# Perception4D/LidarSlam

Hardware: AMD Instinct MI355X
Metric: LiDAR frames/sec (AddFrame end-to-end), VLS-128 scan (higher is better)
Workload: dtype f32+f64; 1 GPU; VLS-128 synthetic spinning scan, street canyon, 5 m/s, EgoMotion=MOTION_EXTRAPOLATION_AND_REGISTRATION, Undistortion=REFINED, library defaults; points_per_frame=255802, sequences=1, parallelism=1 sequence per GPU x 1, frames_resident_in_hbm=False

## Files before the change

include/lidarslam_amd.h:

```cpp
#ifndef LIDARSLAM_AMD_H
#define LIDARSLAM_AMD_H

#include <stddef.h>
#include <stdint.h>

#ifdef __cplusplus
extern "C" {
#endif

#define LSA_OK 0
#define LSA_E_NO_DEVICE (-1)
#define LSA_E_HIP (-2)
#define LSA_E_ARG (-3)
#define LSA_E_STATE (-4)
#define LSA_E_CAPACITY (-5)

#define LSA_EDGE 0
#define LSA_PLANE 1
#define LSA_BLOB 2

typedef struct lsa_point_t
{
  float x, y, z, w;
  double time;
// ... 118 lines not shown
int lsa_stage_target_ahead(lsa_ctx* ctx, int slot, int type, int m);
int lsa_drop_target_ahead(lsa_ctx* ctx, int slot, int type);
int lsa_staged_targets_adopted(const lsa_ctx* ctx);
int lsa_set_target_from_set(lsa_ctx* ctx, int slot, int type, int set);
int lsa_prepare_previous_targets(lsa_ctx* ctx, unsigned type_mask);
int lsa_prepared_targets_adopted(const lsa_ctx* ctx);
int lsa_target_size(const lsa_ctx* ctx, int slot, int type);
int lsa_download_target(lsa_ctx* ctx, int slot, int type, lsa_point_t* out, int capacity);
int lsa_set_target_cell_size(lsa_ctx* ctx, int slot, int type, float cell);
int lsa_set_knn_lanes(lsa_ctx* ctx, int type, int lanes);
int lsa_set_knn_rounds(lsa_ctx* ctx, int type, int rounds);

long long lsa_match_serial(const lsa_ctx* ctx, int type);
int lsa_match_histogram(lsa_ctx* ctx, int type, long long serial, int histogram[LSA_MATCH_NSTATUS]);
int lsa_match_types_undistorted(lsa_ctx* ctx, int slot, unsigned type_mask, const lsa_match_params_t* p, const double pose[16], int* histograms,
                                const double H0[16], const double H1[16], double t0, double t1);
int lsa_set_fused_match(lsa_ctx* ctx, int on);
int lsa_match_slow_queries(lsa_ctx* ctx);
int lsa_match_route_stats(lsa_ctx* ctx, int type, int out[8]);
int lsa_match_trace(lsa_ctx* ctx, unsigned long long* out, int blocks);
int lsa_match_exhaustive_queries(lsa_ctx* ctx);

int lsa_set_keypoints(lsa_ctx* ctx, int set, int type, const lsa_point_t* pts, int k);

int lsa_match(lsa_ctx* ctx, int slot, int type, int query_set, const lsa_match_params_t* params, const double pose[16],
              int histogram[LSA_MATCH_NSTATUS]);

int lsa_match_types(lsa_ctx* ctx, int slot, unsigned type_mask, int query_set, const lsa_match_params_t* params, const double pose[16],
                    int* histograms);

int lsa_overlap(lsa_ctx* ctx, unsigned type_mask, int interpolate, const double H0[16], const double H1[16], double t0, double t1, float sampling_ratio,
                const double leaf_size[3], float* overlap);

int lsa_download_match(lsa_ctx* ctx, int type, uint8_t* status, double* weights, double* records, int capacity);
int lsa_upload_match(lsa_ctx* ctx, int type, const uint8_t* status, const double* records, int n, double saturation);
#define LSA_KNN_MAX 16
int lsa_download_knn(lsa_ctx* ctx, int type, int* idx, float* d2, int* cnt, int capacity);

int lsa_accumulate(lsa_ctx* ctx, unsigned type_mask, const double w[6], int want_jacobian, double* cost, double g[6],
                   double H[36], int* n_valid);
int lsa_mailbox_active(const lsa_ctx* ctx);

int lsa_solve(lsa_ctx* ctx, unsigned type_mask, const double prior[16], int lm_max_iter, int two_d_mode, double optimized[16],
              int summary[4], double costs[2]);
typedef struct lsa_solve_result
{
  double pose[6];
  double initial_cost, final_cost;
  double cost, g[6], H[36];
  int num_successful_steps;
  int num_unsuccessful_steps;
  int num_iterations;
  int num_evaluations;
  int num_matches;
  int skipped;
  int termination;
  const char* message;
} lsa_solve_result_t;
int lsa_solve_device(lsa_ctx* ctx, unsigned type_mask, const double prior[6], int two_d_mode, int lm_max_iter, int min_matches,
                     lsa_solve_result_t* out);
int lsa_solve_device_begin(lsa_ctx* ctx, unsigned type_mask, const double prior[6], int two_d_mode, int lm_max_iter, int min_matches);
int lsa_solve_device_end(lsa_ctx* ctx, lsa_solve_result_t* out);
int lsa_solve_device_drop(lsa_ctx* ctx);

int lsa_icp_cancel(lsa_ctx* ctx, int ticket);
int lsa_icp_abandon(lsa_ctx* ctx);
int lsa_match_types_linked(lsa_ctx* ctx, int slot, unsigned type_mask, int query_set, const lsa_match_params_t* p, int undistort);
typedef struct lsa_icp_link
{
  int refine_undistortion;
  int first;
  int have_log;
  double prev_time, cur_time;
  double max_extrapolation_ratio;
  double previous_world[16];
  double motion[16];
} lsa_icp_link_t;
int lsa_icp_link(lsa_ctx* ctx);
int lsa_solve_device_begin_linked(lsa_ctx* ctx, unsigned type_mask, const double prior[6], int two_d_mode, int lm_max_iter, int min_matches,
                                  int leave_ticket, const lsa_icp_link_t* link);
int lsa_icp_link_peek(lsa_ctx* ctx, int ticket, unsigned long long words[64]);
int lsa_icp_link_expected(const double x[6], int skipped, int successful_steps, const lsa_icp_link_t* link, unsigned long long words[64], double motion_after[16]);

int lsa_solve_device_trace(lsa_ctx* ctx, unsigned long long out[12]);
int lsa_debug_set(lsa_ctx* ctx, const char* name, int value);
int lsa_solve_device_shape(const lsa_ctx* ctx, int out[4]);
int lsa_accumulate_shape(const lsa_ctx* ctx, int out[4]);
int lsa_solve_device_fallbacks(const lsa_ctx* ctx);
int lsa_solve_device_interlude(lsa_ctx* ctx, void (*fn)(void*), void* arg);
int lsa_registration_error(lsa_ctx* ctx, unsigned type_mask, const double pose[16], int two_d_mode, double cov[36], double err[2]);

typedef struct lsa_sensor_terms_t
{
  int wheel;
  double wheel_weight;
  double p[3];
  double d;
  int gravity;
  double gravity_weight;
  double g_ref[3];
  double g_cur[3];
} lsa_sensor_terms_t;
int lsa_set_sensor_terms(lsa_ctx* ctx, const lsa_sensor_terms_t* terms);
int lsa_sensor_terms_eval(const lsa_sensor_terms_t* terms, const double w[6], double sums[29]);

typedef struct lsa_sensors lsa_sensors;
lsa_sensors* lsa_sensors_create(void);
void lsa_sensors_destroy(lsa_sensors* s);
int lsa_sensors_add_wheel_odom(lsa_sensors* s, double time, double distance);
int lsa_sensors_add_gravity(lsa_sensors* s, double time, const double acc[3]);
int lsa_sensors_set_weights(lsa_sensors* s, double wheel_weight, double gravity_weight);
int lsa_sensors_set_time_offset(lsa_sensors* s, double offset);
int lsa_sensors_clear(lsa_sensors* s);
int lsa_sensors_compute(lsa_sensors* s, double lidar_time, lsa_sensor_terms_t* out);
int lsa_sensors_gravity_ref(const lsa_sensors* s, double g[3]);


int lsa_reset_working_keypoints(lsa_ctx* ctx);

int lsa_undistort(lsa_ctx* ctx, const double H0[16], const double H1[16], double t0, double t1);

int lsa_localization_begin(lsa_ctx* ctx, const double H0[16], const double H1[16], double t0, double t1, const double box_pose[16]);
int lsa_arm_localization_boxes(lsa_ctx* ctx);

int lsa_working_time_range(lsa_ctx* ctx, double* tmin, double* tmax);
int lsa_keypoint_time_range(lsa_ctx* ctx, int set, double* tmin, double* tmax);
int lsa_working_bbox(lsa_ctx* ctx, int type, const double pose[16], float mn[3], float mx[3]);
int lsa_working_bboxes(lsa_ctx* ctx, const double pose[16], float mn[9], float mx[9]);
int lsa_keypoint_bboxes_begin(lsa_ctx* ctx, int set, const double pose[16]);
int lsa_keypoint_bboxes_begin_interp(lsa_ctx* ctx, int set, const double H0[16], const double H1[16], double t0, double t1);
int lsa_keypoint_bboxes_end(lsa_ctx* ctx, float mn[9], float mx[9]);
int lsa_keypoint_boxes_predicted_mark(lsa_ctx* ctx);
int lsa_keypoint_boxes_predicted(lsa_ctx* ctx, int set, const double H0[16], const double H1[16], double t0, double t1);

int lsa_download_transformed(lsa_ctx* ctx, int set, int type, const double pose[16], lsa_point_t* out, int capacity);
int lsa_stage_transformed(lsa_ctx* ctx, int set, const double pose[16]);
int lsa_staged_transformed(lsa_ctx* ctx, int type, const lsa_point_t** pts, int* n);

int lsa_transform_frame(lsa_ctx* ctx, int interpolate, const double H0[16], const double H1[16], double t0, double t1,
                        lsa_point_t* out, int capacity);
int lsa_transform_frame_at(lsa_ctx* ctx, int interpolate, const double H0[16], const double H1[16], double t0, double t1, double time_offset,
                           lsa_point_t* out, int capacity);

int lsa_selftest_math(lsa_ctx* ctx, int fn, const double* x, const double* y, int n, double* out);
int lsa_selftest_numerics(lsa_ctx* ctx, int fn, const double* in, int n, double* out);
int lsa_selftest_lm_step(lsa_ctx* ctx, int n_scripts, const int* header, const double* x0, const double* sums, double* records, double* results, int* status);
int lsa_selftest_lm_host(int n_scripts, const int* header, const double* x0, const double* sums, double* records, double* results, int* status);
int lsa_selftest_labels(lsa_ctx* ctx, const lsa_extract_params_t* params, const int* ring_lengths, int nrings, const float* sin_angle,
                        const float* depth_gap, const float* saliency, const float* intensity_gap, const uint8_t* valid,
                        uint8_t* label_out, uint8_t* valid_out, int* ring_counts_out);
int lsa_selftest_keep_busy(lsa_ctx* ctx, int ms, int blocks);

typedef struct lsa_kernel_stat_t
{
  char name[48];
  uint32_t launches;
  double total_ms;
  double bytes;
} lsa_kernel_stat_t;
int lsa_profile_enable(lsa_ctx* ctx, int on);
double lsa_profile_event_overhead_us(const lsa_ctx* ctx);
int lsa_profile_select(lsa_ctx* ctx, const char* scope, int every);
int lsa_profile_reset(lsa_ctx* ctx);
int lsa_profile_get(lsa_ctx* ctx, lsa_kernel_stat_t* out, int capacity);

typedef struct lsa_slam lsa_slam;

// ... 447 lines not shown
```

lidarslam_amd/_context.py:

```python
import ctypes as C

import numpy as np

from ._abi import E_STATE, KNN_MAX, TARGET_MAP, TARGET_PREVIOUS, LsaError, SolveResult, _error, lib
from ._native import MATCH_NSTATUS, POINT_DTYPE, SET_WORKING, ExtractParams, KernelStat, pose16, ptr
from ._place import PlaceParams
from ._pose_graph import (
    pose_graph_assemble,
    pose_graph_linearize,
    pose_graph_linearize_priors,
    pose_graph_premultiply,
    pose_graph_reanchor,
    pose_graph_retract,
    pose_graph_solve,
    pose_graph_spmv,
    pose_graph_tridiagonal_solve,
)

DEBUG_NAMES = [
    "sin_angle", "saliency", "depth_gap", "intensity_gap", "edge_keypoint", "plane_keypoint", "blob_keypoint",
    "edge_validity", "plane_validity", "blob_validity",
]


# ... 247 lines not shown
            self.L.lsa_download_match(self.h, ktype, ptr(status), ptr(weights), ptr(rec) if records else None, n), "lsa_download_match"
        )
        return status[:got], weights[:got], (rec[:got] if records else None)

    def route_stats(self, ktype):
        out = np.zeros(8, np.int32)
        self._check(self.L.lsa_match_route_stats(self.h, ktype, ptr(out)), "lsa_match_route_stats")
        return out

    def match_trace(self, blocks):
        out = np.zeros((blocks, 12), np.uint64)
        self._check(self.L.lsa_match_trace(self.h, ptr(out), blocks), "lsa_match_trace")
        return out

    def set_fused_match(self, on):
        self._check(self.L.lsa_set_fused_match(self.h, int(on)), "lsa_set_fused_match")

    def slow_queries(self):
        return self.L.lsa_match_slow_queries(self.h)

    def accumulate(self, type_mask, w, jac=True):
        w = np.ascontiguousarray(w, np.float64)
        cost = C.c_double()
        nv = C.c_int()
        g = np.zeros(6)
        H = np.zeros((6, 6))
        self._check(self.L.lsa_accumulate(self.h, type_mask, ptr(w), int(jac), C.byref(cost), ptr(g), ptr(H), C.byref(nv)), "lsa_accumulate")
        return cost.value, g, H, nv.value

    def solve(self, type_mask, prior, max_iter=15, two_d=False):
        out = np.zeros(16)
        summ = np.zeros(4, np.int32)
        costs = np.zeros(2)
        self._check(self.L.lsa_solve(self.h, type_mask, ptr(pose16(prior)), max_iter, int(two_d), ptr(out), ptr(summ), ptr(costs)), "lsa_solve")
        return out.reshape(4, 4), summ, costs

    def solve_device(self, type_mask, prior6, max_iter=15, two_d=False, min_matches=0):
        r = SolveResult()
        w = np.ascontiguousarray(prior6, np.float64)
        self._check(self.L.lsa_solve_device(self.h, type_mask, ptr(w), int(two_d), max_iter, min_matches, C.byref(r)), "lsa_solve_device")
        return r

    def solve_device_begin(self, type_mask, prior6=None, max_iter=15, two_d=False, min_matches=0):
        w = None if prior6 is None else np.ascontiguousarray(prior6, np.float64)
        self._check(self.L.lsa_solve_device_begin(self.h, type_mask, None if w is None else ptr(w), int(two_d), max_iter, min_matches), "lsa_solve_device_begin")

    def solve_device_end(self):
        r = SolveResult()
        rc = self.L.lsa_solve_device_end(self.h, C.byref(r))
        return r if rc == 0 else rc

    def solve_device_drop(self):
        self._check(self.L.lsa_solve_device_drop(self.h), "lsa_solve_device_drop")

    def icp_link(self):
        return self._check(self.L.lsa_icp_link(self.h), "lsa_icp_link")

    def solve_device_begin_linked(self, type_mask, prior6, leave_ticket, link, max_iter=15, two_d=False, min_matches=0):
        w = None if prior6 is None else np.ascontiguousarray(prior6, np.float64)
        self._check(self.L.lsa_solve_device_begin_linked(self.h, type_mask, None if w is None else ptr(w), int(two_d), max_iter, min_matches, leave_ticket,
                                                         None if link is None else C.byref(link)), "lsa_solve_device_begin_linked")

    def icp_link_peek(self, ticket):
        out = np.zeros(64, np.uint64)
        self._check(self.L.lsa_icp_link_peek(self.h, ticket, ptr(out)), "lsa_icp_link_peek")
        return out

    def icp_cancel(self, ticket):
        self._check(self.L.lsa_icp_cancel(self.h, ticket), "lsa_icp_cancel")

    def icp_abandon(self):
        self._check(self.L.lsa_icp_abandon(self.h), "lsa_icp_abandon")

    def match_types_linked(self, type_mask, query_set, params, undistort=False, slot=TARGET_MAP):
        return self._check(self.L.lsa_match_types_linked(self.h, slot, type_mask, query_set, C.byref(params), int(undistort)), "lsa_match_types_linked")

    def profile_event_overhead_us(self):
        return float(self.L.lsa_profile_event_overhead_us(self.h))

    def debug_set(self, name, value):
        self._check(self.L.lsa_debug_set(self.h, name.encode(), int(value)), "lsa_debug_set")

    def solve_device_trace(self):
        out = np.zeros(12, np.uint64)
        self._check(self.L.lsa_solve_device_trace(self.h, ptr(out)), "lsa_solve_device_trace")
        return out

    def solve_device_fallbacks(self):
        return self.L.lsa_solve_device_fallbacks(self.h)

    def solve_device_shape(self):
        out = np.zeros(4, np.int32)
        self._check(self.L.lsa_solve_device_shape(self.h, ptr(out)), "lsa_solve_device_shape")
        return tuple(int(v) for v in out)

    def accumulate_shape(self):
        out = np.zeros(4, np.int32)
        self._check(self.L.lsa_accumulate_shape(self.h, ptr(out)), "lsa_accumulate_shape")
        return tuple(int(v) for v in out)

    def set_sensor_terms(self, terms=None):
        self._check(self.L.lsa_set_sensor_terms(self.h, C.byref(terms) if terms is not None else None), "lsa_set_sensor_terms")

    def registration_error(self, type_mask, pose, two_d=False):
        cov = np.zeros((6, 6))
        err = np.zeros(2)
        self._check(self.L.lsa_registration_error(self.h, type_mask, ptr(pose16(pose)), int(two_d), ptr(cov), ptr(err)), "lsa_registration_error")
        return cov, err

    def selftest_math(self, fn, x, y=None):
        x = np.ascontiguousarray(x, np.float64)
        y = np.ascontiguousarray(x if y is None else y, np.float64)
        out = np.zeros_like(x)
        self._check(self.L.lsa_selftest_math(self.h, fn, ptr(x), ptr(y), x.size, ptr(out)), "lsa_selftest_math")
        return out

    def selftest_numerics(self, fn, records):
        return selftest_numerics(fn, records, self)

    def selftest_labels(self, ring_lengths, sin_angle, depth_gap, saliency, intensity_gap, valid, params=None):
        params = params or ExtractParams()
        lens = np.ascontiguousarray(ring_lengths, np.int32)
        n = int(lens.sum())
        scores = [np.ascontiguousarray(a, np.float32) for a in (sin_angle, depth_gap, saliency, intensity_gap)]
        valid = np.ascontiguousarray(valid, np.uint8)
        assert all(a.size == n for a in scores) and valid.size == n
        label, after, counts = np.zeros(n, np.uint8), np.zeros(n, np.uint8), np.zeros((lens.size, 3), np.int32)
        self._check(self.L.lsa_selftest_labels(self.h, C.byref(params), ptr(lens), lens.size, *[ptr(a) for a in scores], ptr(valid), ptr(label),
                                               ptr(after), ptr(counts)), "lsa_selftest_labels")
        return label, after, counts

    def reset_working_keypoints(self):
        self._check(self.L.lsa_reset_working_keypoints(self.h), "lsa_reset_working_keypoints")

    def undistort(self, H0, H1, t0, t1):
        self._check(self.L.lsa_undistort(self.h, ptr(pose16(H0)), ptr(pose16(H1)), t0, t1), "lsa_undistort")

    def localization_begin(self, H0=None, H1=None, t0=0.0, t1=0.0, box_pose=None, arm=False):
        if arm:
            self._check(self.L.lsa_arm_localization_boxes(self.h), "lsa_arm_localization_boxes")
        self._check(self.L.lsa_localization_begin(self.h, ptr(pose16(H0)) if H0 is not None else None, ptr(pose16(H1)) if H1 is not None else None,
                                                  C.c_double(t0), C.c_double(t1), ptr(pose16(box_pose)) if box_pose is not None else None), "lsa_localization_begin")

    def keypoint_bboxes_end(self):
        mn, mx = np.zeros(9, np.float32), np.zeros(9, np.float32)
        self._check(self.L.lsa_keypoint_bboxes_end(self.h, ptr(mn), ptr(mx)), "lsa_keypoint_bboxes_end")
        return mn.reshape(3, 3), mx.reshape(3, 3)

    def working_time_range(self):
        a, b = C.c_double(), C.c_double()
        self._check(self.L.lsa_working_time_range(self.h, C.byref(a), C.byref(b)), "lsa_working_time_range")
        return a.value, b.value

    def keypoint_time_range(self, kset):
        a, b = C.c_double(), C.c_double()
        self._check(self.L.lsa_keypoint_time_range(self.h, kset, C.byref(a), C.byref(b)), "lsa_keypoint_time_range")
        return a.value, b.value

    def keypoint_bboxes(self, kset, H0, H1=None, t0=0.0, t1=0.0):
        if H1 is None:
            self._check(self.L.lsa_keypoint_bboxes_begin(self.h, kset, ptr(pose16(H0))), "lsa_keypoint_bboxes_begin")
        else:
            self._check(self.L.lsa_keypoint_bboxes_begin_interp(self.h, kset, ptr(pose16(H0)), ptr(pose16(H1)), C.c_double(t0), C.c_double(t1)),
                        "lsa_keypoint_bboxes_begin_interp")
        mn, mx = np.zeros(9, np.float32), np.zeros(9, np.float32)
        self._check(self.L.lsa_keypoint_bboxes_end(self.h, ptr(mn), ptr(mx)), "lsa_keypoint_bboxes_end")
        return mn.reshape(3, 3), mx.reshape(3, 3)
# ... 159 lines not shown
```

lidarslam_amd/csrc/lsa_lm.hip:

```cpp
#include <chrono>
#include <cmath>
#include "lsa_accum.h"
#include "lsa_device_math.h"
#include "lsa_sensor_terms.h"
#include "../../include/lsa_pmath.h"

using namespace lsa;

namespace
{

typedef unsigned long long u64;
#ifndef LSA_RECORD_PREFETCH
#define LSA_RECORD_PREFETCH 1
#endif
constexpr bool kRecordPrefetch = LSA_RECORD_PREFETCH != 0;

struct LmParams
{
  RecordSet set;
  double x0[6];
  int two_d;
  int max_iter;
  int min_matches;
  unsigned tag_base;
  int cslots;
  int give_up_block;
  const IcpLinkBlock* link;
  IcpLinkBlock* leave;
  int link_refine;
  int motion_from_args;
  posemath::ScanPoseClock clock;
  Rigid previous_world;
  double motion0[16];
  double* motion_dev;
  lsa_sensor_terms_t sensors;
  int sensors_on;
};

constexpr int kResPose = 0, kResInitial = 6, kResFinal = 7, kResSums = 8, kResSuccessful = 37, kResUnsuccessful = 38, kResIterations = 39,
              kResEvaluations = 40, kResSkipped = 41, kResCode = 42, kResMatches = 43, kResFailed = 44, kResCount = 45;
static_assert(kResCount <= kLmOut, "result does not fit the mailbox");

__device__ __forceinline__ constexpr int hidx(int a, int b) { return 7 + a * 6 - (a * (a - 1)) / 2 + (b - a); }
__device__ __forceinline__ constexpr int hsym(int a, int b) { return a <= b ? hidx(a, b) : hidx(b, a); }

struct LmState
{
  int cur_buf;
  double x[6], scale[6], diag[6];
  double radius, decrease_factor, x_norm, model_cost_change, delta_norm, initial_cost;
  int reuse_diagonal, consecutive_invalid, iter;
  int evaluations, successful, unsuccessful, iterations, code, skipped, matches;
};

struct Shared
{
  double wsum[kLmThreads / 64][kAccumVals];
  double part[kAccumVals][8];
  double sums[2][kAccumVals];
  double Hs[36], gs[6];
  double w[6];
  double rot[39];
  LmState lm;
  int failed;
  int stop;
  unsigned long long lap[6], tk;
  unsigned long long sub[4], st0;
};

__device__ __forceinline__ double uniform(double v)
{
  const long long b = __double_as_longlong(v);
  const int lo = __builtin_amdgcn_readfirstlane((int)(b & 0xffffffffll)), hi = __builtin_amdgcn_readfirstlane((int)(b >> 32));
  return __longlong_as_double(((long long)hi << 32) | (long long)(unsigned)lo);
}

__device__ __forceinline__ double lane_value(double v, int lane)
{
  const long long b = __double_as_longlong(v);
  const int lo = __shfl((int)(b & 0xffffffffll), lane), hi = __shfl((int)(b >> 32), lane);
  return __longlong_as_double(((long long)hi << 32) | (long long)(unsigned)lo);
}

__device__ __forceinline__ double lane_bcast(double v, int src)
{
  const long long b = __double_as_longlong(v);
  const int lo = __builtin_amdgcn_readlane((int)(b & 0xffffffffll), src), hi = __builtin_amdgcn_readlane((int)(b >> 32), src);
  return __longlong_as_double(((long long)hi << 32) | (long long)(unsigned)lo);
}

__device__ __forceinline__ void lm_lap(Shared& sh, int slot)
{
  if (threadIdx.x == 0)
  {
    const unsigned long long now = wall_clock64();
    sh.lap[slot] += now - sh.tk;
    sh.tk = now;
  }
}

__device__ __noinline__ void lm_sensor_terms(const lsa_sensor_terms_t* terms, Shared& sh)
{
  sensor_terms_add(*terms, sh.w, sh.rot, sh.rot + 9, sh.rot + 18, sh.rot + 27, true, sh.sums[1 - sh.lm.cur_buf]);
}

__device__ __forceinline__ bool lm_evaluate(const LmParams& p, unsigned epoch, u64* __restrict__ xchg, Shared& sh, double* __restrict__ cache, bool trace)
{
  {
    RotConst c;
#pragma unroll
    for (int i = 0; i < 9; ++i) { c.R[i] = uniform(sh.rot[i]); c.dRx[i] = uniform(sh.rot[9 + i]); c.dRy[i] = uniform(sh.rot[18 + i]); c.dRz[i] = uniform(sh.rot[27 + i]); }
#pragma unroll
    for (int i = 0; i < 3; ++i) c.t[i] = uniform(sh.rot[36 + i]);
    double acc[kAccumVals];
#pragma unroll
    for (int v = 0; v < kAccumVals; ++v) acc[v] = 0.;
    const unsigned long long e0 = trace ? wall_clock64() : 0ull;
    accumulate_records_cached(p.set, c, blockIdx.x * blockDim.x + threadIdx.x, gridDim.x * blockDim.x, cache, p.cslots, p.cslots * kLmThreads, epoch == 1, kRecordPrefetch && p.cslots > 0 ? 1 : 0, acc);
    const unsigned long long e1 = trace ? wall_clock64() : 0ull;
    int slot;
    const double total = wave_reduce_accum(acc, slot);
    if (trace && threadIdx.x == 0) { sh.lap[4] += e1 - e0; }
    if ((threadIdx.x & 1) == 0 && slot < kAccumVals) sh.wsum[threadIdx.x >> 6][slot] = total;
  }
  if (threadIdx.x == 0) sh.failed = 0;
  __syncthreads();
  if (trace) lm_lap(sh, 0);
  const unsigned tag = p.tag_base + epoch;
  const int nb = gridDim.x;
  u64* slots = xchg + (size_t)(epoch & 1u) * kLmBlocksMax * kMailboxStride;
  if (threadIdx.x < 2 * kAccumVals)
  {
    const int v = threadIdx.x >> 1, half = threadIdx.x & 1;
    double r = sh.wsum[0][v];
#pragma unroll
    for (int w = 1; w < kLmThreads / 64; ++w) r += sh.wsum[w][v];
    const u64 bits = (u64)__double_as_longlong(r);
    const unsigned word = half ? (unsigned)(bits >> 32) : (unsigned)(bits & 0xffffffffull);
    __hip_atomic_store(slots + (size_t)blockIdx.x * kMailboxStride + threadIdx.x, ((u64)tag << 32) | word, __ATOMIC_RELAXED, __HIP_MEMORY_SCOPE_AGENT);
  }
  static_assert(kLmThreads / 64 == 8, "a wavefront per partial sum of the fold");
  bool failed = (int)blockIdx.x == p.give_up_block;
  {
    constexpr int kFoldBatch = 8;
    const int j = threadIdx.x >> 6, s = threadIdx.x & 63;
    const bool loads = s < 2 * kAccumVals;
    const u64* mine = slots + s;
    double sum = 0.;
    const unsigned long long t0 = wall_clock64();
    unsigned spins = 0;
// ... 257 lines not shown
#pragma unroll
    for (int j = 0; j < N; ++j)
    {
      const double d = lane_bcast(s[j], j);
      if (!(d > 0.0) || !isfinite(d)) ok = false;
      rinv[j] = 1.0 / __builtin_sqrt(d);
      const double lij = s[j] * rinv[j];
#pragma unroll
      for (int jj = j + 1; jj <= N; ++jj) Lu[jj][j] = lane_bcast(lij, jj);
#pragma unroll
      for (int jj = j + 1; jj < N; ++jj) s[jj] -= lij * Lu[jj][j];
    }
    double y[N];
#pragma unroll
    for (int i = N - 1; i >= 0; --i)
    {
      double t = Lu[N][i];
#pragma unroll
      for (int k = i + 1; k < N; ++k) t -= Lu[k][i] * y[k];
      y[i] = t * rinv[i];
    }
#pragma unroll
    for (int i = 0; i < N; ++i)
      if (!isfinite(y[i])) ok = false;
    stamp(2);
    reuse_diagonal = 1;
    double step[N], t_row = 0, sg = 0, sHs = 0;
#pragma unroll
    for (int a = 0; a < N; ++a) step[a] = -y[a];
#pragma unroll
    for (int b = 0; b < N; ++b) t_row += Hrow[b] * step[b];
#pragma unroll
    for (int a = 0; a < N; ++a)
    {
      sg += step[a] * gs[a];
      sHs += step[a] * lane_bcast(t_row, a);
    }
    const double change = -sg - 0.5 * sHs;
    if (!ok || change < 0.0)
    {
      ++unsuccessful;
      if (++consecutive_invalid >= max_consecutive_invalid) { code = kCodeInvalidSteps; break; }
      radius /= decrease_factor; decrease_factor *= 2.0;
      continue;
    }
    consecutive_invalid = 0;
    model_cost_change = change;
    double dn = 0;
#pragma unroll
    for (int a = 0; a < 6; ++a) cand[a] = x[a];
#pragma unroll
    for (int a = 0; a < N; ++a)
    {
      cand[lm_act<N>(a)] = x[lm_act<N>(a)] + step[a] * scale[a];
      const double e = x[lm_act<N>(a)] - cand[lm_act<N>(a)];
      dn += e * e;
    }
    delta_norm = __builtin_sqrt(dn);
    ++evaluations;
    break;
  }

  if (lane < N) lm.diag[lane] = diag_row;
  if (l0)
  {
    if (use_tot && !first)
    {
#pragma unroll
      for (int a = 0; a < 6; ++a) lm.x[a] = x[a];
    }
    lm.cur_buf = cur_buf;
    lm.x_norm = x_norm; lm.radius = radius; lm.decrease_factor = decrease_factor;
    lm.model_cost_change = model_cost_change; lm.delta_norm = delta_norm;
    lm.reuse_diagonal = reuse_diagonal; lm.consecutive_invalid = consecutive_invalid;
    lm.iter = iter; lm.iterations = iter;
    lm.successful = successful; lm.unsuccessful = unsuccessful; lm.evaluations = evaluations;
    lm.code = code;
    sh.stop = code != kCodeNone ? 1 : 0;
  }
  stamp(3);
  return code != kCodeNone;
}

__device__ void leave_link(const LmParams& p, const LmState& lm, bool failed, int part)
{
  using namespace posemath;
  IcpLinkBlock* g = p.leave;
  const int lane = threadIdx.x & 63;
  const bool go = !failed && !lm.skipped && lm.successful != 1;
  if (!go)
  {
    if (lane == 0 && part == 0) g->go = 0ull;
    return;
  }
  if (part == 1 && !p.link_refine) return;
  const double half = lm.x[3 + (lane < 6 ? lane % 3 : 0)] * 0.5;
  const double v = lane < 3 ? lsa_cos(half) : lsa_sin(half);
  const double cx = lane_value(v, 0), cy = lane_value(v, 1), cz = lane_value(v, 2);
  const double sx = lane_value(v, 3), sy = lane_value(v, 4), sz = lane_value(v, 5);
  double x[6];
#pragma unroll
  for (int a = 0; a < 6; ++a) x[a] = lm.x[a];
  const Pose T = FromXYZRPYTrig(x, cx, sx, cy, sy, cz, sz);
  if (part == 0)
  {
    if (lane != 0) return;
    double x0[6];
    ToXYZRPY(T, x0);
    g->in.pose = ToRigid(T);
#pragma unroll
    for (int a = 0; a < 6; ++a) g->in.x0[a] = x0[a];
    g->go = 1ull;
    return;
  }
  WithinFrameMotion m;
  double mv[16];
#pragma unroll
  for (int i = 0; i < 16; ++i) mv[i] = p.motion0[i];
  if (!p.motion_from_args)
  {
#pragma unroll
    for (int i = 0; i < 16; ++i) mv[i] = p.motion_dev[i];
  }
  m.Time0 = mv[0]; m.Time1 = mv[1];
  m.Rot0 = {mv[2], mv[3], mv[4], mv[5]};
  m.Rot1 = {mv[6], mv[7], mv[8], mv[9]};
#pragma unroll
  for (int i = 0; i < 3; ++i) { m.Trans0[i] = mv[10 + i]; m.Trans1[i] = mv[13 + i]; }
  const Pose previous = FromRigid(p.previous_world);
  const Pose mine = InterpolateScanPose(p.clock, previous, T, lane == 1 ? m.Time1 : m.Time0);
  Pose worldToBaseEnd = Pose::Identity();
#pragma unroll
  for (int i = 0; i < 3; ++i)
#pragma unroll
    for (int j = 0; j < 4; ++j) worldToBaseEnd(i, j) = lane_value(mine(i, j), 1);
  if (lane != 0) return;
  Pose d0, d1;
  RefineUndistortionFrom(m, mine, worldToBaseEnd, T, d0, d1);
  g->in.ic = MakeInterpConst(d0, d1, m.Time0, m.Time1);
  double* o = p.motion_dev;
  o[0] = m.Time0; o[1] = m.Time1;
  o[2] = m.Rot0.w; o[3] = m.Rot0.x; o[4] = m.Rot0.y; o[5] = m.Rot0.z;
  o[6] = m.Rot1.w; o[7] = m.Rot1.x; o[8] = m.Rot1.y; o[9] = m.Rot1.z;
#pragma unroll
  for (int i = 0; i < 3; ++i) { o[10 + i] = m.Trans0[i]; o[13 + i] = m.Trans1[i]; }
}

__global__ __launch_bounds__(kLmThreads) void k_lm_solve(LmParams p, u64* __restrict__ xchg, u64* __restrict__ mailbox, unsigned out_tag, unsigned long long* trace)
{
  __shared__ Shared sh;
  extern __shared__ double lm_cache[];
  const bool tr = trace != nullptr && blockIdx.x == 0;
  RecordRegs pre;
  if (kRecordPrefetch && p.cslots > 0) record_load(p.set, blockIdx.x * blockDim.x + threadIdx.x, pre);
  if (p.link)
  {
    if (p.link->go != 1ull)
    {
      if (p.leave && blockIdx.x == 0 && threadIdx.x == 0) p.leave->go = 0ull;
      return;
    }
  }
  if (threadIdx.x < 64)
  {
    double x0[6];
#pragma unroll
    for (int a = 0; a < 6; ++a) x0[a] = p.x0[a];
    if (p.link)
    {
#pragma unroll
      for (int a = 0; a < 6; ++a) x0[a] = p.link->in.x0[a];
    }
    if (threadIdx.x == 0)
    {
      for (int i = 0; i < 6; ++i) sh.lap[i] = 0;
      for (int i = 0; i < 4; ++i) sh.sub[i] = 0;
      sh.st0 = 0;
      sh.tk = wall_clock64();
      sh.lap[5] = sh.tk;
      LmState& lm = sh.lm;
#pragma unroll
      for (int v = 0; v < kAccumVals; ++v) sh.sums[0][v] = 0.;
      lm.cur_buf = 0;
#pragma unroll
      for (int a = 0; a < 6; ++a) { lm.x[a] = x0[a]; lm.scale[a] = 1.; lm.diag[a] = 0.; }
      lm.radius = 1e4; lm.decrease_factor = 2.0; lm.x_norm = 0.; lm.model_cost_change = 0.; lm.delta_norm = 0.; lm.initial_cost = 0.;
      lm.reuse_diagonal = 0; lm.consecutive_invalid = 0; lm.iter = 0;
      lm.evaluations = 1; lm.successful = 0; lm.unsuccessful = 0; lm.iterations = 0; lm.code = kCodeNone; lm.skipped = 0; lm.matches = 0;
      sh.stop = 0;
    }
    finish_point(sh, x0[0], x0[1], x0[2], x0[3], x0[4], x0[5]);
  }
  if (kRecordPrefetch && p.cslots > 0) record_stash(pre, lm_cache, p.cslots * kLmThreads, threadIdx.x);
  __syncthreads();
  bool failed = false;
  for (unsigned epoch = 1;; ++epoch)
  {
    if (!lm_evaluate(p, epoch, xchg, sh, lm_cache, tr)) { failed = true; break; }
    if (threadIdx.x < 64)
    {
      if (threadIdx.x == 0 && tr) sh.st0 = wall_clock64();
      double cand[6];
      const bool stop = p.two_d ? lm_step<3>(p, sh, epoch == 1, cand) : lm_step<6>(p, sh, epoch == 1, cand);
      if (!stop) finish_point(sh, cand[0], cand[1], cand[2], cand[3], cand[4], cand[5]);
    }
    __syncthreads();
    if (tr) lm_lap(sh, 3);
    if (sh.stop) break;
  }
  if (blockIdx.x != 0) return;
  if (tr && threadIdx.x == 0)
  {
    for (int i = 0; i < 4; ++i) trace[i] += sh.lap[i];
    trace[4] += (unsigned long long)sh.lm.evaluations;
    trace[5] += wall_clock64() - sh.lap[5];
    trace[6] += 1;
    trace[7] += sh.lap[4];
    for (int i = 0; i < 4; ++i) trace[8 + i] += sh.sub[i];
  }
  if (p.leave && threadIdx.x >= 64 && threadIdx.x < 192) leave_link(p, sh.lm, failed, (threadIdx.x >> 6) - 1);
  if (threadIdx.x < 2 * kResCount)
  {
    const LmState& lm = sh.lm;
    const int v = threadIdx.x >> 1, half = threadIdx.x & 1;
    double r = 0.;
    if (v < kResInitial) r = lm.x[v - kResPose];
    else if (v == kResInitial) r = lm.initial_cost;
    else if (v == kResFinal) r = sh.sums[lm.cur_buf][0];
    else if (v < kResSums + kAccumVals) r = sh.sums[lm.cur_buf][v - kResSums];
    else if (v == kResSuccessful) r = lm.successful;
    else if (v == kResUnsuccessful) r = lm.unsuccessful;
    else if (v == kResIterations) r = lm.iterations;
    else if (v == kResEvaluations) r = lm.evaluations;
    else if (v == kResSkipped) r = lm.skipped;
    else if (v == kResCode) r = lm.code;
    else if (v == kResMatches) r = lm.matches;
    else if (v == kResFailed) r = failed ? 1. : 0.;
    const u64 bits = (u64)__double_as_longlong(r);
    const unsigned word = half ? (unsigned)(bits >> 32) : (unsigned)(bits & 0xffffffffull);
    __hip_atomic_store(mailbox + threadIdx.x, ((u64)out_tag << 32) | word, __ATOMIC_RELAXED, __HIP_MEMORY_SCOPE_SYSTEM);
  }
}

constexpr int kStepRecord = 42;
__global__ __launch_bounds__(64) void k_selftest_lm_step(const int* __restrict__ header, const int* __restrict__ first_eval, const double* __restrict__ x0s,
                                                         const double* __restrict__ sums, double* __restrict__ records, double* __restrict__ results,
                                                         int* __restrict__ status)
{
  __shared__ Shared sh;
  const int s = blockIdx.x;
  const int two_d = header[4 * s], evals = header[4 * s + 3];
  const size_t first = (size_t)first_eval[s];
  LmParams p;
  p.max_iter = header[4 * s + 1];
  p.min_matches = header[4 * s + 2];
  {
    double x0[6];
#pragma unroll
    for (int a = 0; a < 6; ++a) x0[a] = x0s[(size_t)s * 6 + a];
    if (threadIdx.x == 0)
    {
      for (int i = 0; i < 6; ++i) sh.lap[i] = 0;
      for (int i = 0; i < 4; ++i) sh.sub[i] = 0;
      sh.st0 = 0;
      sh.tk = 0;
      LmState& lm = sh.lm;
#pragma unroll
      for (int v = 0; v < kAccumVals; ++v) sh.sums[0][v] = 0.;
      lm.cur_buf = 0;
#pragma unroll
      for (int a = 0; a < 6; ++a) { lm.x[a] = x0[a]; lm.scale[a] = 1.; lm.diag[a] = 0.; }
      lm.radius = 1e4; lm.decrease_factor = 2.0; lm.x_norm = 0.; lm.model_cost_change = 0.; lm.delta_norm = 0.; lm.initial_cost = 0.;
      lm.reuse_diagonal = 0; lm.consecutive_invalid = 0; lm.iter = 0;
      lm.evaluations = 1; lm.successful = 0; lm.unsuccessful = 0; lm.iterations = 0; lm.code = kCodeNone; lm.skipped = 0; lm.matches = 0;
      sh.stop = 0;
      sh.failed = 0;
    }
    finish_point(sh, x0[0], x0[1], x0[2], x0[3], x0[4], x0[5]);
  }
  __syncthreads();
  int used = 0;
  bool stopped = false;
  while (used < evals && !stopped)
  {
    if (threadIdx.x < kAccumVals) sh.sums[1 - sh.lm.cur_buf][threadIdx.x] = sums[(first + used) * kAccumVals + threadIdx.x];
    asm volatile("s_waitcnt lgkmcnt(0)" ::: "memory");
    double cand[6];
    const bool stop = two_d ? lm_step<3>(p, sh, used == 0, cand) : lm_step<6>(p, sh, used == 0, cand);
    if (!stop) finish_point(sh, cand[0], cand[1], cand[2], cand[3], cand[4], cand[5]);
    __syncthreads();
    if (threadIdx.x == 0)
    {
      const LmState& lm = sh.lm;
      double* o = records + (first + used) * kStepRecord;
#pragma unroll
      for (int a = 0; a < 6; ++a) o[a] = stop ? 0. : cand[a];
      o[6] = lm.code; o[7] = sh.stop;
      o[8] = lm.radius; o[9] = lm.decrease_factor; o[10] = lm.x_norm; o[11] = lm.model_cost_change; o[12] = lm.delta_norm; o[13] = lm.initial_cost;
      o[14] = lm.reuse_diagonal; o[15] = lm.consecutive_invalid; o[16] = lm.iter; o[17] = lm.evaluations; o[18] = lm.successful;
      o[19] = lm.unsuccessful; o[20] = lm.iterations; o[21] = lm.skipped; o[22] = lm.matches;
      for (int a = 0; a < 6; ++a) { o[23 + a] = lm.x[a]; o[29 + a] = lm.scale[a]; o[35 + a] = lm.diag[a]; }
      o[41] = lm.cur_buf;
    }
    ++used;
    stopped = sh.stop != 0;
    __syncthreads();
  }
  if (threadIdx.x == 0) { status[2 * s] = stopped ? 0 : 1; status[2 * s + 1] = used; }
  if (threadIdx.x < kResCount)
  {
    const LmState& lm = sh.lm;
    const int v = threadIdx.x;
    double r = 0.;
    if (v < kResInitial) r = lm.x[v - kResPose];
    else if (v == kResInitial) r = lm.initial_cost;
    else if (v == kResFinal) r = sh.sums[lm.cur_buf][0];
    else if (v < kResSums + kAccumVals) r = sh.sums[lm.cur_buf][v - kResSums];
    else if (v == kResSuccessful) r = lm.successful;
    else if (v == kResUnsuccessful) r = lm.unsuccessful;
    else if (v == kResIterations) r = lm.iterations;
    else if (v == kResEvaluations) r = lm.evaluations;
    else if (v == kResSkipped) r = lm.skipped;
    else if (v == kResCode) r = lm.code;
// ... 333 lines not shown
  else if (n == "mailbox_check") ctx->mailbox_check = value < 0 ? c.mailbox_check : value != 0;
  else if (n == "pcd_lds") ctx->pcd_lds = value < 0 ? -1 : (value != 0);
  else if (n == "kplog_chunk_kib") ctx->kplog_chunk_bytes = value < 0 ? ((size_t)32 << 20) : (size_t)std::max(value, 1) << 10;
  else if (n == "kplog_fail_alloc") ctx->debug_kplog_fail_alloc = value > 0 ? 1 : 0;
  else if (n == "place_max_blocks") ctx->place_max_blocks = value > 0 ? value : 0;
  else if (n == "place_untiled") ctx->place_untiled = value != 0;
  else if (n == "place_table_bytes") ctx->place_table_bytes = value > 0 ? value : 0;
  else if (n == "map_describe_slice") ctx->map_describe_slice = value > 0 ? value : 0;
  else if (n == "map_describe_cull") ctx->map_describe_cull = value != 0;
  else return ctx->fail(LSA_E_ARG, "lsa_debug_set: no such knob");
  return LSA_OK;
}

int lsa_solve_device_shape(const lsa_ctx* ctx, int out[4])
{
  if (!ctx || !out) return LSA_E_ARG;
  std::memcpy(out, ctx->lm_shape, sizeof(ctx->lm_shape));
  return LSA_OK;
}

int lsa_accumulate_shape(const lsa_ctx* ctx, int out[4])
{
  if (!ctx || !out) return LSA_E_ARG;
  std::memcpy(out, ctx->accum_shape, sizeof(ctx->accum_shape));
  return LSA_OK;
}

int lsa_solve_device_fallbacks(const lsa_ctx* ctx) { return ctx ? ctx->lm_fallbacks : 0; }

int lsa_set_sensor_terms(lsa_ctx* ctx, const lsa_sensor_terms_t* terms)
{
  if (!ctx) return LSA_E_ARG;
  if (terms) ctx->sensor_terms = *terms;
  else std::memset(&ctx->sensor_terms, 0, sizeof(ctx->sensor_terms));
  return LSA_OK;
}

int lsa_solve_device_interlude(lsa_ctx* ctx, void (*fn)(void*), void* arg)
{
  if (!ctx) return LSA_E_ARG;
  ctx->solve_hook = fn;
  ctx->solve_hook_arg = arg;
  return LSA_OK;
}

int lsa_selftest_lm_step(lsa_ctx* ctx, int n_scripts, const int* header, const double* x0, const double* sums, double* records, double* results, int* status)
{
  if (!ctx) return LSA_E_ARG;
  if (n_scripts <= 0 || n_scripts > 65536 || !header || !x0 || !sums || !records || !results || !status) return ctx->fail(LSA_E_ARG, "lsa_selftest_lm_step: bad argument");
  std::vector<int> first(n_scripts);
  size_t total = 0;
  for (int s = 0; s < n_scripts; ++s)
  {
    if (header[4 * s + 1] < 0 || header[4 * s + 3] < 1 || header[4 * s + 3] > 4096) return ctx->fail(LSA_E_ARG, "lsa_selftest_lm_step: a script needs max_iter >= 0 and 1 to 4096 evaluations");
    first[s] = (int)total;
    total += (size_t)header[4 * s + 3];
  }
  LSA_HIP(ctx, hipSetDevice(ctx->device));
  const size_t n = (size_t)n_scripts;
  const size_t doubles = n * 6 + total * kAccumVals + total * kStepRecord + n * kResCount, ints = n * 4 + n + n * 2;
  const int rc = ensure_scratch(ctx, doubles * sizeof(double) + ints * sizeof(int));
  if (rc) return rc;
  double* d_x0 = (double*)ctx->scratch_out;
  double* d_sums = d_x0 + n * 6;
  double* d_records = d_sums + total * kAccumVals;
  double* d_results = d_records + total * kStepRecord;
  int* d_header = (int*)(d_results + n * kResCount);
  int* d_first = d_header + n * 4;
  int* d_status = d_first + n;
  LSA_HIP(ctx, hipMemcpyAsync(d_x0, x0, n * 6 * sizeof(double), hipMemcpyHostToDevice, ctx->stream));
  LSA_HIP(ctx, hipMemcpyAsync(d_sums, sums, total * kAccumVals * sizeof(double), hipMemcpyHostToDevice, ctx->stream));
  LSA_HIP(ctx, hipMemcpyAsync(d_header, header, n * 4 * sizeof(int), hipMemcpyHostToDevice, ctx->stream));
  LSA_HIP(ctx, hipMemcpyAsync(d_first, first.data(), n * sizeof(int), hipMemcpyHostToDevice, ctx->stream));
  LSA_HIP(ctx, hipMemsetAsync(d_records, 0, total * kStepRecord * sizeof(double), ctx->stream));
  hipLaunchKernelGGL(k_selftest_lm_step, dim3(n_scripts), dim3(64), 0, ctx->stream, d_header, d_first, d_x0, d_sums, d_records, d_results, d_status);
  LSA_HIP(ctx, hipGetLastError());
  LSA_HIP(ctx, hipMemcpyAsync(records, d_records, total * kStepRecord * sizeof(double), hipMemcpyDeviceToHost, ctx->stream));
  LSA_HIP(ctx, hipMemcpyAsync(results, d_results, n * kResCount * sizeof(double), hipMemcpyDeviceToHost, ctx->stream));
  LSA_HIP(ctx, hipMemcpyAsync(status, d_status, n * 2 * sizeof(int), hipMemcpyDeviceToHost, ctx->stream));
  LSA_HIP(ctx, hipStreamSynchronize(ctx->stream));
  return LSA_OK;
}

int lsa_solve_device_trace(lsa_ctx* ctx, unsigned long long out[12])
{
  if (!ctx || !out || !ctx->trace_dev) return LSA_E_ARG;
  if (hipStreamSynchronize(ctx->stream) != hipSuccess) return LSA_E_HIP;
  if (hipMemcpy(out, reinterpret_cast<unsigned long long*>(ctx->trace_dev) + (size_t)8192 * 12, 12 * sizeof(unsigned long long), hipMemcpyDeviceToHost) != hipSuccess) return LSA_E_HIP;
  return LSA_OK;
}

}
```

Measured before the change: 1398 frames/s.

## Overlap ICP link pose staging with LM iterations on idle waves

Moves the computation of the next-solve link inputs (pose and Euler x0) out of the kernel tail. Idle waves now compute them speculatively during each LM epoch into double-buffered shared staging, and only a word copy is committed at the end. The state initialisation is also hoisted before the go-check, and the link x0 load is overlapped with the record prefetch. The change adds trace marks (trace buffer widened to 16 words) and shared memory, and it relies on the buffer index tracking cur_buf correctly.

```diff
diff --git a/include/lidarslam_amd.h b/include/lidarslam_amd.h
--- a/include/lidarslam_amd.h
+++ b/include/lidarslam_amd.h
@@ -224,7 +224,7 @@
 int lsa_icp_link_peek(lsa_ctx* ctx, int ticket, unsigned long long words[64]);
 int lsa_icp_link_expected(const double x[6], int skipped, int successful_steps, const lsa_icp_link_t* link, unsigned long long words[64], double motion_after[16]);
 
-int lsa_solve_device_trace(lsa_ctx* ctx, unsigned long long out[12]);
+int lsa_solve_device_trace(lsa_ctx* ctx, unsigned long long out[16]);
 int lsa_debug_set(lsa_ctx* ctx, const char* name, int value);
 int lsa_solve_device_shape(const lsa_ctx* ctx, int out[4]);
 int lsa_accumulate_shape(const lsa_ctx* ctx, int out[4]);
diff --git a/lidarslam_amd/_context.py b/lidarslam_amd/_context.py
--- a/lidarslam_amd/_context.py
+++ b/lidarslam_amd/_context.py
@@ -353,7 +353,7 @@
         self._check(self.L.lsa_debug_set(self.h, name.encode(), int(value)), "lsa_debug_set")
 
     def solve_device_trace(self):
-        out = np.zeros(12, np.uint64)
+        out = np.zeros(16, np.uint64)
         self._check(self.L.lsa_solve_device_trace(self.h, ptr(out)), "lsa_solve_device_trace")
         return out
 
diff --git a/lidarslam_amd/csrc/lsa_lm.hip b/lidarslam_amd/csrc/lsa_lm.hip
--- a/lidarslam_amd/csrc/lsa_lm.hip
+++ b/lidarslam_amd/csrc/lsa_lm.hip
@@ -54,6 +54,12 @@
   int evaluations, successful, unsuccessful, iterations, code, skipped, matches;
 };
 
+struct LinkStage
+{
+  Rigid pose;
+  double x0[6];
+};
+
 struct Shared
 {
   double wsum[kLmThreads / 64][kAccumVals];
@@ -63,10 +69,14 @@
   double w[6];
   double rot[39];
   LmState lm;
+  LinkStage stage[2];
+  double link_w[2][6];
+  int link_buf;
   int failed;
   int stop;
   unsigned long long lap[6], tk;
   unsigned long long sub[4], st0;
+  unsigned long long mark[4];
 };
 
 __device__ __forceinline__ double uniform(double v)
@@ -490,37 +500,63 @@
   return code != kCodeNone;
 }
 
-__device__ void leave_link(const LmParams& p, const LmState& lm, bool failed, int part)
+__device__ __forceinline__ posemath::Pose link_pose(const double* xs, int lane)
+{
+  const double half = xs[3 + (lane < 6 ? lane % 3 : 0)] * 0.5;
+  const double v = lane < 3 ? lsa_cos(half) : lsa_sin(half);
+  const double cx = lane_bcast(v, 0), cy = lane_bcast(v, 1), cz = lane_bcast(v, 2);
+  const double sx = lane_bcast(v, 3), sy = lane_bcast(v, 4), sz = lane_bcast(v, 5);
+  double x[6];
+#pragma unroll
+  for (int a = 0; a < 6; ++a) x[a] = xs[a];
+  return posemath::FromXYZRPYTrig(x, cx, sx, cy, sy, cz, sz);
+}
+
+__device__ __noinline__ void link_start(const double* xs, LinkStage& out)
 {
   using namespace posemath;
+  const int lane = threadIdx.x & 63, half = (threadIdx.x >> 6) - 1;
+  const Pose T = link_pose(xs, lane);
+  if (half == 1)
+  {
+    if (lane != 0) return;
+    out.pose = ToRigid(T);
+#pragma unroll
+    for (int a = 0; a < 3; ++a) out.x0[a] = T(a, 3);
+    out.x0[4] = -lsa_asin(T(2, 0));
+    return;
+  }
+  if (lane >= 2) return;
+  const double angle = lsa_atan2(lane == 0 ? T(2, 1) : T(1, 0), lane == 0 ? T(2, 2) : T(0, 0));
+  out.x0[lane == 0 ? 3 : 5] = angle;
+}
+
+__device__ __forceinline__ bool link_goes(const LmState& lm, bool failed) { return !failed && !lm.skipped && lm.successful != 1; }
+
+__device__ __forceinline__ void link_commit(const LmParams& p, const Shared& sh, bool failed)
+{
+  constexpr int kStartWords = (int)(sizeof(LinkStage) / 8);
+  static_assert(offsetof(IcpLinkBlock, in) == 8 && offsetof(IcpInputs, pose) == 0 && offsetof(IcpInputs, x0) == sizeof(Rigid) &&
+                offsetof(LinkStage, x0) == sizeof(Rigid) && kStartWords == 18, "the staged words are the block's words 1 to 18");
+  const int lane = threadIdx.x & 63;
+  u64* g = reinterpret_cast<u64*>(p.leave);
+  if (!link_goes(sh.lm, failed))
+  {
+    if (lane == 0) g[0] = 0ull;
+    return;
+  }
+  const u64* words = reinterpret_cast<const u64*>(&sh.stage[sh.lm.cur_buf]);
+  if (lane == 0) g[0] = 1ull;
+  else if (lane <= kStartWords) g[lane] = words[lane - 1];
+}
+
+__device__ void link_refine(const LmParams& p, const LmState& lm, bool failed)
+{
+  using namespace posemath;
+  if (!link_goes(lm, failed)) return;
   IcpLinkBlock* g = p.leave;
   const int lane = threadIdx.x & 63;
-  const bool go = !failed && !lm.skipped && lm.successful != 1;
-  if (!go)
-  {
-    if (lane == 0 && part == 0) g->go = 0ull;
-    return;
-  }
-  if (part == 1 && !p.link_refine) return;
-  const double half = lm.x[3 + (lane < 6 ? lane % 3 : 0)] * 0.5;
-  const double v = lane < 3 ? lsa_cos(half) : lsa_sin(half);
-  const double cx = lane_value(v, 0), cy = lane_value(v, 1), cz = lane_value(v, 2);
-  const double sx = lane_value(v, 3), sy = lane_value(v, 4), sz = lane_value(v, 5);
-  double x[6];
-#pragma unroll
-  for (int a = 0; a < 6; ++a) x[a] = lm.x[a];
-  const Pose T = FromXYZRPYTrig(x, cx, sx, cy, sy, cz, sz);
-  if (part == 0)
-  {
-    if (lane != 0) return;
-    double x0[6];
-    ToXYZRPY(T, x0);
-    g->in.pose = ToRigid(T);
-#pragma unroll
-    for (int a = 0; a < 6; ++a) g->in.x0[a] = x0[a];
-    g->go = 1ull;
-    return;
-  }
+  const Pose T = link_pose(lm.x, lane);
   WithinFrameMotion m;
   double mv[16];
 #pragma unroll
@@ -559,48 +595,65 @@
   __shared__ Shared sh;
   extern __shared__ double lm_cache[];
   const bool tr = trace != nullptr && blockIdx.x == 0;
+  if (tr && threadIdx.x == 0) sh.mark[0] = wall_clock64();
   RecordRegs pre;
   if (kRecordPrefetch && p.cslots > 0) record_load(p.set, blockIdx.x * blockDim.x + threadIdx.x, pre);
+  const bool links = p.leave != nullptr && blockIdx.x == 0;
+  u64 go = 1ull;
+  double x0[6];
+#pragma unroll
+  for (int a = 0; a < 6; ++a) x0[a] = p.x0[a];
   if (p.link)
   {
-    if (p.link->go != 1ull)
-    {
-      if (p.leave && blockIdx.x == 0 && threadIdx.x == 0) p.leave->go = 0ull;
-      return;
-    }
-  }
+    go = p.link->go;
+    if (threadIdx.x < 64)
+    {
+#pragma unroll
+      for (int a = 0; a < 6; ++a) x0[a] = p.link->in.x0[a];
+    }
+  }
+  if (threadIdx.x == 0)
+  {
+    for (int i = 0; i < 6; ++i) sh.lap[i] = 0;
+    for (int i = 0; i < 4; ++i) sh.sub[i] = 0;
+    sh.st0 = 0;
+    LmState& lm = sh.lm;
+#pragma unroll
+    for (int v = 0; v < kAccumVals; ++v) sh.sums[0][v] = 0.;
+    lm.cur_buf = 0;
+#pragma unroll
+    for (int a = 0; a < 6; ++a) { lm.scale[a] = 1.; lm.diag[a] = 0.; }
+    lm.radius = 1e4; lm.decrease_factor = 2.0; lm.x_norm = 0.; lm.model_cost_change = 0.; lm.delta_norm = 0.; lm.initial_cost = 0.;
+    lm.reuse_diagonal = 0; lm.consecutive_invalid = 0; lm.iter = 0;
+    lm.evaluations = 1; lm.successful = 0; lm.unsuccessful = 0; lm.iterations = 0; lm.code = kCodeNone; lm.skipped = 0; lm.matches = 0;
+    sh.stop = 0;
+  }
+  if (go != 1ull)
+  {
+    if (links && threadIdx.x == 0) p.leave->go = 0ull;
+    return;
+  }
+  if (tr && threadIdx.x == 0) sh.mark[1] = wall_clock64();
   if (threadIdx.x < 64)
   {
-    double x0[6];
-#pragma unroll
-    for (int a = 0; a < 6; ++a) x0[a] = p.x0[a];
-    if (p.link)
-    {
-#pragma unroll
-      for (int a = 0; a < 6; ++a) x0[a] = p.link->in.x0[a];
-    }
     if (threadIdx.x == 0)
     {
-      for (int i = 0; i < 6; ++i) sh.lap[i] = 0;
-      for (int i = 0; i < 4; ++i) sh.sub[i] = 0;
-      sh.st0 = 0;
       sh.tk = wall_clock64();
       sh.lap[5] = sh.tk;
-      LmState& lm = sh.lm;
-#pragma unroll
-      for (int v = 0; v < kAccumVals; ++v) sh.sums[0][v] = 0.;
-      lm.cur_buf = 0;
-#pragma unroll
-      for (int a = 0; a < 6; ++a) { lm.x[a] = x0[a]; lm.scale[a] = 1.; lm.diag[a] = 0.; }
-      lm.radius = 1e4; lm.decrease_factor = 2.0; lm.x_norm = 0.; lm.model_cost_change = 0.; lm.delta_norm = 0.; lm.initial_cost = 0.;
-      lm.reuse_diagonal = 0; lm.consecutive_invalid = 0; lm.iter = 0;
-      lm.evaluations = 1; lm.successful = 0; lm.unsuccessful = 0; lm.iterations = 0; lm.code = kCodeNone; lm.skipped = 0; lm.matches = 0;
-      sh.stop = 0;
+#pragma unroll
+      for (int a = 0; a < 6; ++a) sh.lm.x[a] = x0[a];
+      if (links)
+      {
+#pragma unroll
+        for (int a = 0; a < 6; ++a) sh.link_w[1][a] = x0[a];
+        sh.link_buf = 1;
+      }
     }
     finish_point(sh, x0[0], x0[1], x0[2], x0[3], x0[4], x0[5]);
   }
   if (kRecordPrefetch && p.cslots > 0) record_stash(pre, lm_cache, p.cslots * kLmThreads, threadIdx.x);
   __syncthreads();
+  if (tr && threadIdx.x == 0) sh.mark[3] = wall_clock64();
   bool failed = false;
   for (unsigned epoch = 1;; ++epoch)
   {
@@ -610,23 +663,27 @@
       if (threadIdx.x == 0 && tr) sh.st0 = wall_clock64();
       double cand[6];
       const bool stop = p.two_d ? lm_step<3>(p, sh, epoch == 1, cand) : lm_step<6>(p, sh, epoch == 1, cand);
-      if (!stop) finish_point(sh, cand[0], cand[1], cand[2], cand[3], cand[4], cand[5]);
+      if (!stop)
+      {
+        finish_point(sh, cand[0], cand[1], cand[2], cand[3], cand[4], cand[5]);
+        if (links && threadIdx.x == 0)
+        {
+#pragma unroll
+          for (int a = 0; a < 6; ++a) sh.link_w[(epoch + 1) & 1u][a] = cand[a];
+        }
+      }
+    }
+    else if (links && threadIdx.x < 192)
+    {
+      link_start(sh.link_w[epoch & 1u], sh.stage[sh.link_buf]);
     }
     __syncthreads();
     if (tr) lm_lap(sh, 3);
     if (sh.stop) break;
+    if (links && threadIdx.x == 64) sh.link_buf = 1 - sh.lm.cur_buf;
   }
   if (blockIdx.x != 0) return;
-  if (tr && threadIdx.x == 0)
-  {
-    for (int i = 0; i < 4; ++i) trace[i] += sh.lap[i];
-    trace[4] += (unsigned long long)sh.lm.evaluations;
-    trace[5] += wall_clock64() - sh.lap[5];
-    trace[6] += 1;
-    trace[7] += sh.lap[4];
-    for (int i = 0; i < 4; ++i) trace[8 + i] += sh.sub[i];
-  }
-  if (p.leave && threadIdx.x >= 64 && threadIdx.x < 192) leave_link(p, sh.lm, failed, (threadIdx.x >> 6) - 1);
+  if (tr && threadIdx.x == 0) sh.mark[2] = wall_clock64();
   if (threadIdx.x < 2 * kResCount)
   {
     const LmState& lm = sh.lm;
@@ -647,6 +704,26 @@
     const u64 bits = (u64)__double_as_longlong(r);
     const unsigned word = half ? (unsigned)(bits >> 32) : (unsigned)(bits & 0xffffffffull);
     __hip_atomic_store(mailbox + threadIdx.x, ((u64)out_tag << 32) | word, __ATOMIC_RELAXED, __HIP_MEMORY_SCOPE_SYSTEM);
+  }
+  if (links && threadIdx.x >= 64 && threadIdx.x < 128) link_commit(p, sh, failed);
+  if (links && p.link_refine && threadIdx.x >= 128 && threadIdx.x < 192) link_refine(p, sh.lm, failed);
+  if (tr)
+  {
+    __syncthreads();
+    if (threadIdx.x == 0)
+    {
+      const unsigned long long last = wall_clock64();
+      for (int i = 0; i < 4; ++i) trace[i] += sh.lap[i];
+      trace[4] += (unsigned long long)sh.lm.evaluations;
+      trace[5] += sh.mark[2] - sh.lap[5];
+      trace[6] += 1;
+      trace[7] += sh.lap[4];
+      for (int i = 0; i < 4; ++i) trace[8 + i] += sh.sub[i];
+      trace[12] += sh.mark[1] - sh.mark[0];
+      trace[13] += sh.mark[3] - sh.mark[0];
+      trace[14] += last - sh.mark[2];
+      trace[15] += last - sh.mark[0];
+    }
   }
 }
 
@@ -1146,12 +1223,12 @@
   return LSA_OK;
 }
 
-int lsa_solve_device_trace(lsa_ctx* ctx, unsigned long long out[12])
+int lsa_solve_device_trace(lsa_ctx* ctx, unsigned long long out[16])
 {
   if (!ctx || !out || !ctx->trace_dev) return LSA_E_ARG;
   if (hipStreamSynchronize(ctx->stream) != hipSuccess) return LSA_E_HIP;
-  if (hipMemcpy(out, reinterpret_cast<unsigned long long*>(ctx->trace_dev) + (size_t)8192 * 12, 12 * sizeof(unsigned long long), hipMemcpyDeviceToHost) != hipSuccess) return LSA_E_HIP;
-  return LSA_OK;
-}
-
-}
+  if (hipMemcpy(out, reinterpret_cast<unsigned long long*>(ctx->trace_dev) + (size_t)8192 * 12, 16 * sizeof(unsigned long long), hipMemcpyDeviceToHost) != hipSuccess) return LSA_E_HIP;
+  return LSA_OK;
+}
+
+}
```

After: 1384 frames/s. 1.0% lower.
